# NicholasMilef/UUO-Mocap

Hardware: AMD Instinct MI355X
Metric: mocap frames/sec fitted (300-frame seq, 50 markers) (higher is better)
Workload: dtype f32

## Files before the change

### uuo_mocap_amd/csrc/closure.hip

```cpp
#include <cstddef>
#include <cstdlib>
#include <cstring>
#include <vector>

#include "frame_math.h"
#include "tri_math.h"

#define UUO_STAGE_UPSTREAM 3

struct FinArgs {
  UuoGridHdr h;
  int stage, F;
  uuo_gptr<const float> frame_part;
  uuo_gptr<const float> betas;
  uuo_gptr<const float> o_betas;
  double closs;
  double cpose;
  double cbetas;
  uuo_gptr<float> g_betas;
  uuo_gptr<float> g_z;
  uuo_gptr<float> loss;
  uuo_gptr<const float> dir_betas;
  uuo_gptr<const float> dir_z;
  uuo_gptr<double> stats;
// ... 274 lines not shown
        FIN_REP(12, __double_as_longlong(own1));
        FIN_REP(13, __double_as_longlong(own2));
#pragma unroll
        for (int l = 0; l < 10; ++l) FIN_REP(14 + l, __double_as_longlong((double)gb_local[l]));
#undef FIN_REP
        if constexpr (COHERENT) {
          asm volatile("s_waitcnt vmcnt(0)" ::: "memory");
          __hip_atomic_store(&a.rep_host[10], a.rep_seq, __ATOMIC_RELAXED, __HIP_MEMORY_SCOPE_SYSTEM);
        } else {
          __threadfence_system();
          __hip_atomic_store(&a.rep_host[10], a.rep_seq, __ATOMIC_RELEASE, __HIP_MEMORY_SCOPE_SYSTEM);
        }
      }
    }
  }
}

#ifdef UUO_DEBUG_HOOKS
#define BWD_NSTAMP 12
__device__ unsigned long long g_bwd_stamps[4096 * BWD_NSTAMP];
#define BWD_STAMP(i)                                                                                          \
  do {                                                                                                        \
    if (a.stop == 9 && threadIdx.x == 0 && blockIdx.x < 4096)                                                 \
      g_bwd_stamps[blockIdx.x * BWD_NSTAMP + (i)] = __builtin_amdgcn_s_memtime();                              \
  } while (0)
#else
#define BWD_STAMP(i) do {} while (0)
#endif
__device__ __forceinline__ float gmof_q(float sig2, float s) { return sig2 / (sig2 + s); }

#define BWD_NW 4
#define BWD_SLOTS (BWD_NW * 4)
#ifndef UUO_FIN_FUSED
#define UUO_FIN_FUSED 0
#endif
#if UUO_FIN_FUSED || defined(UUO_DEBUG_HOOKS)
#define UUO_FIN_FUSED_BUILT 1
#define BWD_FP_STORE(i_, v_) \
  __hip_atomic_store(a.frame_part.get() + (size_t)f * UUO_FP + (i_), (float)(v_), __ATOMIC_RELAXED, __HIP_MEMORY_SCOPE_AGENT)
#else
#define UUO_FIN_FUSED_BUILT 0
#define BWD_FP_STORE(i_, v_) a.frame_part[(size_t)f * UUO_FP + (i_)] = (float)(v_)
#endif
enum : unsigned {
  BWD_PART = 1u << 0,
  BWD_ONE_WAVE = 1u << 1,
  BWD_DENSE = 1u << 2,
  BWD_ITEMS = 1u << 3,
  BWD_ROBUST = 1u << 4,
  BWD_ACCEL = 1u << 5,
  BWD_OFFS = 1u << 6,
  BWD_FASSIGN = 1u << 7,
  BWD_FLOOR = 1u << 8,
};
template <unsigned FL>
__device__ __forceinline__ void bwd_body(const BwdArgs& a) {
  constexpr bool PART = (FL & BWD_PART) != 0, DENSE = (FL & BWD_DENSE) != 0, ITEMS = (FL & BWD_ITEMS) != 0;
  constexpr bool ROBUST = (FL & BWD_ROBUST) != 0, ACCEL = (FL & BWD_ACCEL) != 0, OFFS = (FL & BWD_OFFS) != 0;
  constexpr bool FASSIGN = (FL & BWD_FASSIGN) != 0, FLOOR = (FL & BWD_FLOOR) != 0;
  constexpr int NWV = (FL & BWD_ONE_WAVE) ? 1 : BWD_NW;
  static_assert(!FLOOR || (ACCEL && !(FASSIGN && !ITEMS)), "the floor-contact term rides on the temporal instantiations (slot 3 of "
                "the partials, the frames' FrameLds), outside the per-frame vertex table of the one-hot marker closure");
  static_assert(!FASSIGN || (!OFFS && !PART && !DENSE && NWV == BWD_NW), "per-frame vertex ids belong to item mode (the surface "
                "chamfer closure) and to the marker stage's one-hot closure, without latent offsets");
  static_assert(!OFFS || (!PART && !DENSE && NWV == BWD_NW), "the latent marker offsets are built for the marker stage's "
                "sparse kernels only");
  static_assert(!ROBUST || (!DENSE && !ITEMS), "the robust data term is formed on the sparse items (k_bary_fwd for item mode)");
  static_assert(!ACCEL || (!PART && !DENSE && NWV == BWD_NW), "the joint-acceleration term is built for the fitted stages' "
                "sparse kernels (chamfer, marker) only");
  static_assert(!(PART && DENSE), "the part stage's dense sums come through the runtime `pre` pointer");
  static_assert(!ITEMS || (!PART && !DENSE), "item mode belongs to the general sparse kernel");
  static_assert(NWV == BWD_NW || (PART && NWV == 1), "one-wave blocks exist for the part stage only");
  constexpr int NT = NWV * 64, SLOTS = NWV * 4;
  if constexpr (NWV == BWD_NW) __builtin_amdgcn_s_setprio(2);
  __shared__ FrameLds L;
  __shared__ float sA[UUO_NUM_JOINTS * 12];
  __shared__ float spf[UUO_KB];
  __shared__ float w_dA[SLOTS][UUO_NUM_JOINTS * 12];
  __shared__ float w_dpf[PART ? 1 : SLOTS][PART ? 256 : UUO_KB];
  __shared__ float w_red[SLOTS][16];
  __shared__ float sdA[UUO_NUM_JOINTS * 12];
  __shared__ float sdpf[UUO_KB];
  __shared__ float red[16];
  __shared__ float sdGR[UUO_NUM_JOINTS][9], sdGt[UUO_NUM_JOINTS][3], sdJ[UUO_NUM_JOINTS][3], sdR[UUO_NUM_JOINTS][9];
  __shared__ float spsq[UUO_NUM_JOINTS];
  __shared__ float sstat[28][4];
  __shared__ int s_lvl_n[UUO_MAX_DEPTH], s_lvl_j[UUO_MAX_DEPTH][UUO_LEVEL_W], s_lvl_p[UUO_MAX_DEPTH][UUO_LEVEL_W];
  __shared__ int s_nch[UUO_NUM_JOINTS], s_ch[UUO_NUM_JOINTS][4];
  constexpr int ACC_W = 75, ACC_UJ = 5 * ACC_W, ACC_AA = ACC_UJ + 72;
  __shared__ float s_acc[ACCEL ? ACC_AA + 72 : 1];

  const int f = blockIdx.x;
  const int tid = threadIdx.x, wave = tid >> 6, lane = tid & 63;
  const int F = a.F, M = a.M;
  BWD_STAMP(0);
  {
    const UuoTree* tr_ = a.tree;
    if (tid < UUO_MAX_DEPTH) s_lvl_n[tid] = tr_->level_n[tid];
    if (tid < UUO_MAX_DEPTH * UUO_LEVEL_W) {
      (&s_lvl_j[0][0])[tid] = (&tr_->level_j[0][0])[tid];
      (&s_lvl_p[0][0])[tid] = (&tr_->level_p[0][0])[tid];
    }
    if constexpr (NWV >= 4) {
      if (tid >= 64 && tid < 64 + UUO_NUM_JOINTS) s_nch[tid - 64] = tr_->nchild[tid - 64];
      if (tid >= 128 && tid < 128 + UUO_NUM_JOINTS * 4) (&s_ch[0][0])[tid - 128] = (&tr_->child[0][0])[tid - 128];
    } else {
      if (tid < UUO_NUM_JOINTS) s_nch[tid] = tr_->nchild[tid];
      for (int i = tid; i < UUO_NUM_JOINTS * 4; i += NT) (&s_ch[0][0])[i] = (&tr_->child[0][0])[i];
    }
  }
  if (a.frames) {
    constexpr int NW = sizeof(FrameLds) / 4;
    float* dst_l = reinterpret_cast<float*>(&L);
    for (int i = tid; i < NW; i += NT) dst_l[i] = a.frames[(size_t)f * NW + i];
    __syncthreads();
  } else {
    frame_forward(a.src, a.tree, f, L);
  }
  if constexpr (ACCEL) {
    constexpr int NW = sizeof(FrameLds) / 4, GT = offsetof(FrameLds, Gt) / 4;
    for (int i = tid; i < 5 * ACC_W; i += NT) {
      const int t = i / ACC_W, k = i - t * ACC_W, ft = f - 2 + t;
      float v = 0.f;
      if (ft >= 0 && ft < F) v = (k < 72) ? a.frames[(size_t)ft * NW + GT + k] : a.src.trans[(size_t)ft * 3 + (k - 72)];
      s_acc[i] = v;
    }
    if (a.lock_w != 0.f && tid >= NT - 6) {
      const int q = tid - (NT - 6), sft = q / 3, k = (10 + sft) * 3 + (q - sft * 3);
      const float c0 = a.contacts[(size_t)f * 2 + sft];
      s_acc[ACC_UJ + k] = (f >= 1) ? c0 * a.contacts[(size_t)(f - 1) * 2 + sft] : 0.f;
      s_acc[ACC_AA + k] = (f + 1 < F) ? a.contacts[(size_t)(f + 1) * 2 + sft] * c0 : 0.f;
    }
  }
  if (tid < UUO_NUM_JOINTS) frame_skin_matrix(L, tid, sA + tid * 12);
  if (!PART && tid < UUO_KB) {
    float v = 0.f;
    if (tid < UUO_NUM_POSE_FEATS) {
      const int j = 1 + tid / 9, e = tid % 9;
      v = L.R[j][e] - ((e == 0 || e == 4 || e == 8) ? 1.f : 0.f);
    }
    spf[tid] = v;
  }
  for (int i = tid; i < SLOTS * UUO_NUM_JOINTS * 12; i += NT) (&w_dA[0][0])[i] = 0.f;
  for (int i = tid; i < 28 * 4; i += NT) (&sstat[0][0])[i] = 0.f;
  __syncthreads();

  if (a.stop == 1) return;
  BWD_STAMP(1);
  bool use_pre = DENSE;
  if constexpr (PART) use_pre = a.pre.get() != nullptr;
  if (use_pre) {
    if constexpr (PART) {
      const float* pr = a.pre.get() + (size_t)f * UUO_PRE;
      for (int i = tid; i < UUO_NUM_JOINTS * 12; i += NT) {
        const int jj = i / 12, e = i - jj * 12;
        sdA[i] = ((e & 3) == 3) ? pr[16 + jj * 3 + (e >> 2)] : 0.f;
      }
      if (tid < 14) red[tid] = pr[tid];
    } else if constexpr (DENSE) {
      const float* pr = a.pre.get() + (size_t)f * UUO_PREG;
      for (int i = tid; i < UUO_NUM_JOINTS * 12; i += NT) sdA[i] = pr[16 + i];
      if (tid < 4) red[tid] = pr[tid];
      if (tid < UUO_NUM_POSE_FEATS + UUO_NUM_BETAS) {
        float acc = 0.f;
        const float* pp = a.dpf_part.get() + (size_t)f * UUO_KP + tid;
        for (int cb = 0; cb < UUO_DPF_NCB; ++cb) acc += pp[(size_t)cb * F * UUO_KP];
        if (tid < UUO_NUM_POSE_FEATS) sdpf[tid] = acc;
        else red[4 + tid - UUO_NUM_POSE_FEATS] = acc;
      } else if (tid == UUO_NUM_POSE_FEATS + UUO_NUM_BETAS) {
        sdpf[UUO_NUM_POSE_FEATS] = 0.f;
      }
    }
  } else if constexpr (!DENSE) {
  float tr[3] = {0.f, 0.f, 0.f};
  if (a.src.trans) {
    tr[0] = a.src.trans[(size_t)f * 3];
    tr[1] = a.src.trans[(size_t)f * 3 + 1];
    tr[2] = a.src.trans[(size_t)f * 3 + 2];
  }
  {
    const int gq = lane >> 4, sl = lane & 15;
    const int slot = wave * 4 + gq;
    float fk[13];
#pragma unroll
    for (int t = 0; t < 13; ++t) fk[t] = PART ? 0.f : spf[sl + 16 * t];
    const float beta_s = (sl < 10) ? L.beta[sl] : 0.f;
    float acc_pf[13];
#pragma unroll
    for (int t = 0; t < 13; ++t) acc_pf[t] = 0.f;
    float acc_db16 = 0.f, acc_dt16 = 0.f, acc_loss16 = 0.f;
    float* my_dA = &w_dA[slot][0];
    struct Item16 {
      float p[3][13];
      float x0, x1, x2, wgt, d2, vt0, vt1, vt2, st0, st1, st2;
      int4 wi;
      float4 ww;
      float o[OFFS ? 3 : 1];
      bool fl;
    };
    auto fetch16 = [&](int m, Item16& q) {
      const bool in = m < M;
      const int mm = in ? m : 0;
      float wgt = in ? 1.f : 0.f;
      float d2 = 0.f;
      int vi;
      float up0 = 0.f, up1 = 0.f, up2 = 0.f;
      bool fl = false;
      if constexpr (FLOOR) fl = !in && m < M + a.floor_k;
      if (FLOOR && fl) {
        const int kf = m - M;
        vi = a.floor_vids[kf];
        const float* pu = a.floor_up + ((size_t)f * a.floor_k + kf) * 3;
        up0 = pu[0]; up1 = pu[1]; up2 = pu[2];
        wgt = 1.f;
      } else if constexpr (ITEMS) {
        if constexpr (FASSIGN)
          vi = a.assign[(size_t)f * M + mm];
        else
          vi = a.assign[mm];
        const float* pu = a.up_items + ((size_t)f * M + mm) * 3;
        up0 = pu[0]; up1 = pu[1]; up2 = pu[2];
      } else if (a.stage == UUO_STAGE_UPSTREAM) {
        if (mm < a.V) {
          vi = mm;
          if (a.up_verts) {
            const float* pu = a.up_verts + ((size_t)f * a.V + mm) * 3;
            up0 = pu[0]; up1 = pu[1]; up2 = pu[2];
          }
        } else {
          vi = a.tree->extra_vids[mm - a.V];
          const float* pu = a.up_joints + ((size_t)f * 45 + UUO_NUM_JOINTS + (mm - a.V)) * 3;
          up0 = pu[0]; up1 = pu[1]; up2 = pu[2];
        }
      } else if (a.stage == UUO_STAGE_MARKER) {
        wgt *= a.mask[(size_t)f * M + mm];
        if constexpr (FASSIGN) {
          vi = a.assign[(size_t)f * M + mm];
          if (vi < 0) {
// ... 18 lines not shown
      if constexpr (FLOOR) q.fl = fl;
      if (ITEMS || a.stage == UUO_STAGE_UPSTREAM || (FLOOR && fl)) {
        q.x0 = up0; q.x1 = up1; q.x2 = up2;
      } else {
        const float* px = a.markers + ((size_t)f * M + mm) * 3;
        q.x0 = px[0]; q.x1 = px[1]; q.x2 = px[2];
      }
      if constexpr (PART) {
        const float* pc = a.C + ((size_t)f * a.V + vi) * 3;
        q.vt0 = pc[0];
        q.vt1 = pc[1];
        q.vt2 = pc[2];
      } else {
        const float* pt = a.PT + (size_t)vi * 3 * UUO_KB + sl;
#pragma unroll
        for (int c = 0; c < 3; ++c)
#pragma unroll
          for (int t = 0; t < 13; ++t) q.p[c][t] = pt[c * UUO_KB + 16 * t];
        q.vt0 = a.vt[(size_t)vi * 3];
        q.vt1 = a.vt[(size_t)vi * 3 + 1];
        q.vt2 = a.vt[(size_t)vi * 3 + 2];
      }
      const float* ps = a.ST + (size_t)vi * 30 + (sl < 10 ? sl : 0);
      q.st0 = (sl < 10) ? ps[0] : 0.f;
      q.st1 = (sl < 10) ? ps[10] : 0.f;
      q.st2 = (sl < 10) ? ps[20] : 0.f;
      q.wi = *reinterpret_cast<const int4*>(a.Wi + (size_t)vi * 4);
      q.ww = *reinterpret_cast<const float4*>(a.Ww + (size_t)vi * 4);
      if constexpr (OFFS) {
        const float* po = a.offs + (size_t)(mm / a.offs_k) * 3;
        q.o[0] = po[0]; q.o[1] = po[1]; q.o[2] = po[2];
        if (FLOOR && fl) q.o[0] = q.o[1] = q.o[2] = 0.f;
      }
    };
    auto row_sum = [](float v) {
      v += dpp_rot<0x128>(v);
      v += dpp_rot<0x124>(v);
      v += dpp_rot<0x122>(v);
      v += dpp_rot<0x121>(v);
      return v;
    };
    const int rounds = ((FLOOR ? M + a.floor_k : M) + SLOTS - 1) / SLOTS;
    Item16 cur;
    for (int r = 0; r < rounds; ++r) {
      fetch16(slot + SLOTS * r, cur);
      const float wgt = cur.wgt, d2 = cur.d2;
      float vp[3];
      if constexpr (PART) {
        vp[0] = cur.vt0 + row_sum(cur.st0 * beta_s);
        vp[1] = cur.vt1 + row_sum(cur.st1 * beta_s);
        vp[2] = cur.vt2 + row_sum(cur.st2 * beta_s);
      } else {
        float s0 = 0.f, s1 = 0.f, s2 = 0.f;
#pragma unroll
        for (int t = 0; t < 13; ++t) {
          s0 = fmaf(cur.p[0][t], fk[t], s0);
          s1 = fmaf(cur.p[1][t], fk[t], s1);
          s2 = fmaf(cur.p[2][t], fk[t], s2);
        }
        vp[0] = row_sum(s0) + (cur.vt0 + row_sum(cur.st0 * beta_s));
        vp[1] = row_sum(s1) + (cur.vt1 + row_sum(cur.st1 * beta_s));
        vp[2] = row_sum(s2) + (cur.vt2 + row_sum(cur.st2 * beta_s));
      }
      if constexpr (OFFS) {
        vp[0] += cur.o[0];
        vp[1] += cur.o[1];
        vp[2] += cur.o[2];
      }
      float T[12];
#pragma unroll
      for (int e = 0; e < 12; ++e) T[e] = 0.f;
      const int wj[4] = {cur.wi.x, cur.wi.y, cur.wi.z, cur.wi.w};
      const float ww[4] = {cur.ww.x, cur.ww.y, cur.ww.z, cur.ww.w};
#pragma unroll
      for (int n = 0; n < 4; ++n) {
        const float4* pa4 = reinterpret_cast<const float4*>(sA + wj[n] * 12);
        const float4 r0 = pa4[0], r1 = pa4[1], r2 = pa4[2];
        const float w = ww[n];
        T[0] = fmaf(w, r0.x, T[0]); T[1] = fmaf(w, r0.y, T[1]); T[2] = fmaf(w, r0.z, T[2]); T[3] = fmaf(w, r0.w, T[3]);
        T[4] = fmaf(w, r1.x, T[4]); T[5] = fmaf(w, r1.y, T[5]); T[6] = fmaf(w, r1.z, T[6]); T[7] = fmaf(w, r1.w, T[7]);
        T[8] = fmaf(w, r2.x, T[8]); T[9] = fmaf(w, r2.y, T[9]); T[10] = fmaf(w, r2.z, T[10]); T[11] = fmaf(w, r2.w, T[11]);
      }
      const float vx = fmaf(T[2], vp[2], fmaf(T[1], vp[1], T[0] * vp[0])) + T[3] + tr[0];
      const float vy = fmaf(T[6], vp[2], fmaf(T[5], vp[1], T[4] * vp[0])) + T[7] + tr[1];
      const float vz = fmaf(T[10], vp[2], fmaf(T[9], vp[1], T[8] * vp[0])) + T[11] + tr[2];
      const float dx = cur.x0 - vx, dy = cur.x1 - vy, dz = cur.x2 - vz;
      float g[3];
      float loss_item;
      if (ITEMS || a.stage == UUO_STAGE_UPSTREAM || (FLOOR && cur.fl)) {
        loss_item = 0.f;
        g[0] = wgt * cur.x0; g[1] = wgt * cur.x1; g[2] = wgt * cur.x2;
      } else if (a.stage == UUO_STAGE_MARKER) {
        const float rr = sqrtf((dx * dx + dy * dy) + dz * dz);
        const float e = rr - a.d0;
        float lw = wgt, gw = wgt;
        if constexpr (ROBUST) {
          const float q = gmof_q(a.rs2, e * e);
          lw = wgt * q;
          gw = wgt * (q * q);
        }
        loss_item = lw * (e * e);
        const float sc = (rr > 0.f) ? (-a.cg * gw * e / rr) : 0.f;
        g[0] = sc * dx; g[1] = sc * dy; g[2] = sc * dz;
      } else {
        float lw = wgt, gw = wgt;
        if constexpr (ROBUST) {
          const float q = gmof_q(a.rs2, d2);
          lw = wgt * q;
          gw = wgt * (q * q);
        }
        loss_item = lw * d2;
        const float sc = -a.cg * gw;
        g[0] = sc * dx; g[1] = sc * dy; g[2] = sc * dz;
      }
      float dvp[3];
#pragma unroll
      for (int c = 0; c < 3; ++c) dvp[c] = fmaf(T[8 + c], g[2], fmaf(T[4 + c], g[1], T[c] * g[0]));
      if constexpr (OFFS) {
        const int mi = slot + SLOTS * r;
        if (mi < M && sl < 3) a.offs_part[((size_t)f * M + mi) * 3 + sl] = (sl == 0) ? dvp[0] : ((sl == 1) ? dvp[1] : dvp[2]);
      }
      if constexpr (!PART) {
#pragma unroll
        for (int t = 0; t < 13; ++t)
          acc_pf[t] += fmaf(cur.p[2][t], dvp[2], fmaf(cur.p[1][t], dvp[1], cur.p[0][t] * dvp[0]));
      }
      acc_db16 += fmaf(cur.st2, dvp[2], fmaf(cur.st1, dvp[1], cur.st0 * dvp[0]));
      if (sl < 12) {
        const int rr_ = sl >> 2, cc_ = sl & 3;
        const float gr = (rr_ == 0) ? g[0] : ((rr_ == 1) ? g[1] : g[2]);
        const float pc = (cc_ == 0) ? vp[0] : ((cc_ == 1) ? vp[1] : ((cc_ == 2) ? vp[2] : 1.f));
        const float val = gr * pc;
#pragma unroll
        for (int n = 0; n < 4; ++n) my_dA[wj[n] * 12 + sl] += ww[n] * val;
      }
      acc_dt16 += (sl == 0) ? g[0] : ((sl == 1) ? g[1] : g[2]);
      acc_loss16 += loss_item;
    }
    if constexpr (!PART) {
#pragma unroll
      for (int t = 0; t < 13; ++t) w_dpf[slot][sl + 16 * t] = acc_pf[t];
    }
    if (sl == 0) w_red[slot][0] = acc_loss16;
    if (sl < 3) w_red[slot][1 + sl] = acc_dt16;
    if (sl < 10) w_red[slot][4 + sl] = acc_db16;
  }

  if (a.stop == 2) return;
  BWD_STAMP(2);
  __syncthreads();
  BWD_STAMP(3);
  if constexpr (!PART) {
    if (tid < UUO_KB) {
      float acc = w_dpf[0][tid];
#pragma unroll
      for (int w = 1; w < SLOTS; ++w) acc += w_dpf[w][tid];
      sdpf[tid] = acc;
    }
  }
  for (int i = tid; i < UUO_NUM_JOINTS * 12; i += NT) {
    float acc = w_dA[0][i];
#pragma unroll
    for (int w = 1; w < SLOTS; ++w) acc += w_dA[w][i];
    sdA[i] = acc;
  }
  if (tid < 14) {
    float acc = w_red[0][tid];
#pragma unroll
    for (int w = 1; w < SLOTS; ++w) acc += w_red[w][tid];
    red[tid] = acc;
  }
  }
  __syncthreads();

  if (a.stop == 3) return;
  BWD_STAMP(4);
  const UuoTree* tree = a.tree;
  const int j = tid;
  float dpre[9] = {0.f, 0.f, 0.f, 0.f, 0.f, 0.f, 0.f, 0.f, 0.f};
  if (a.dir) {
    if (tid >= 1 && tid < UUO_NUM_JOINTS && a.off_pose >= 0) {
      const float* pd = a.dir + a.off_pose + ((size_t)f * 23 + (tid - 1)) * a.gs_pose;
#pragma unroll
      for (int e = 0; e < 9; ++e) dpre[e] = (e < 6 || a.gs_pose == 9) ? pd[e] : 0.f;
    } else if (tid == 0) {
      if (a.stage == UUO_STAGE_CHAMFER) dpre[0] = a.dir[a.off_z + f];
      if (a.stage == UUO_STAGE_MARKER) {
        const float* pd = a.dir + a.off_root + (size_t)f * a.gs_root;
#pragma unroll
        for (int e = 0; e < 6; ++e) dpre[e] = pd[e];
      }
    } else if (tid >= 32 && tid < 35) {
      dpre[0] = a.dir[a.off_trans + (size_t)f * 3 + (tid - 32)];
    }
  }

  float raw_pre[9] = {0.f, 0.f, 0.f, 0.f, 0.f, 0.f, 0.f, 0.f, 0.f}, po_pre[9] = {0.f, 0.f, 0.f, 0.f, 0.f, 0.f, 0.f, 0.f, 0.f};
  if (!PART && j >= 1 && j < UUO_NUM_JOINTS && a.g_pose) {
    const float* pr = a.raw_pose + ((size_t)f * 23 + (j - 1)) * 9;
#pragma unroll
    for (int e = 0; e < 9; ++e) raw_pre[e] = pr[e];
    if (a.cpose != 0.f) {
      const float* po = a.o_pose + ((size_t)f * 23 + (j - 1)) * 9;
#pragma unroll
      for (int e = 0; e < 9; ++e) po_pre[e] = po[e];
    }
  }
  for (int t = tid; t < UUO_NUM_JOINTS * 12; t += NT) {
    const int jj = t / 12, e = t - jj * 12;
    if (e < 9) {
      const int r = e / 3, c = e - r * 3;
      sdGR[jj][e] = sdA[jj * 12 + r * 4 + c] - sdA[jj * 12 + r * 4 + 3] * L.J[jj][c];
    } else {
      const int r = e - 9;
      float uj = (a.stage == UUO_STAGE_UPSTREAM && a.up_joints) ? a.up_joints[((size_t)f * 45 + jj) * 3 + r] : 0.f;
      if constexpr (ACCEL) {
        const int k = jj * 3 + r;
        float w[5], tw[5];
#pragma unroll
        for (int i = 0; i < 5; ++i) {
          w[i] = s_acc[i * ACC_W + k];
          tw[i] = s_acc[i * ACC_W + 72 + r];
        }
        float ac[3];
#pragma unroll
        for (int i = 0; i < 3; ++i) {
// ... 29 lines not shown
        const int nch = s_nch[jj];
        const int c0 = s_ch[jj][0], c1 = s_ch[jj][1], c2 = s_ch[jj][2], c3 = s_ch[jj][3];
        if (e < 9) {
          const int r = e / 3, aa = e - r * 3;
          float acc = sdGR[jj][e];
#pragma unroll
          for (int ci = 0; ci < 4; ++ci) {
            if (ci < nch) {
              const int c = (ci == 0) ? c0 : ((ci == 1) ? c1 : ((ci == 2) ? c2 : c3));
              float add = fmaf(sdGR[c][r * 3 + 2], L.R[c][aa * 3 + 2],
                               fmaf(sdGR[c][r * 3 + 1], L.R[c][aa * 3 + 1], sdGR[c][r * 3] * L.R[c][aa * 3]));
              add = fmaf(sdGt[c][r], L.J[c][aa] - L.J[jj][aa], add);
              acc += add;
            }
          }
          sdGR[jj][e] = acc;
        } else {
          const int r = e - 9;
          float acc_t = sdGt[jj][r], acc_j = sdJ[jj][r];
#pragma unroll
          for (int ci = 0; ci < 4; ++ci) {
            if (ci < nch) {
              const int c = (ci == 0) ? c0 : ((ci == 1) ? c1 : ((ci == 2) ? c2 : c3));
              acc_t += sdGt[c][r];
              acc_j -= fmaf(L.GR[jj][6 + r], sdGt[c][2], fmaf(L.GR[jj][3 + r], sdGt[c][1], L.GR[jj][r] * sdGt[c][0]));
            }
          }
          sdGt[jj][r] = acc_t;
          sdJ[jj][r] = acc_j;
        }
      } else if (role == 1 && rl < 12 * UUO_LEVEL_W && k < s_lvl_n[d + 1]) {
        const int jj = s_lvl_j[d + 1][k], p = s_lvl_p[d + 1][k];
        if (e < 9) {
          const int aa = e / 3, bb = e - aa * 3;
          sdR[jj][e] = fmaf(L.GR[p][6 + aa], sdGR[jj][6 + bb], fmaf(L.GR[p][3 + aa], sdGR[jj][3 + bb], L.GR[p][aa] * sdGR[jj][bb]));
        } else {
          const int aa = e - 9;
          sdJ[jj][aa] += fmaf(L.GR[p][6 + aa], sdGt[jj][2], fmaf(L.GR[p][3 + aa], sdGt[jj][1], L.GR[p][aa] * sdGt[jj][0]));
        }
      }
     }
      __syncthreads();
    }
  }
  if (tid < 12) {
    if (tid < 9) sdR[0][tid] = sdGR[0][tid];
    else sdJ[0][tid - 9] += sdGt[0][tid - 9];
  }
  __syncthreads();

  BWD_STAMP(6);
  for (int t = tid; t < 240; t += NT) {
    const int jj = t / 10, l = t - jj * 10;
    w_dpf[0][t] = fmaf(tree->JS[jj][2][l], sdJ[jj][2], fmaf(tree->JS[jj][1][l], sdJ[jj][1], tree->JS[jj][0][l] * sdJ[jj][0]));
  }
  __syncthreads();
  if (tid < 10) {
    float acc = red[4 + tid];
    for (int jj = 0; jj < UUO_NUM_JOINTS; ++jj) acc += w_dpf[0][jj * 10 + tid];
    BWD_FP_STORE(4 + tid, acc);
    if (a.stage == UUO_STAGE_UPSTREAM) a.g_betas_frame[(size_t)f * 10 + tid] = acc;
  }
  BWD_STAMP(7);
  if (j >= 1 && j < UUO_NUM_JOINTS) {
    float psq = 0.f;
    if (!PART && a.g_pose) {
      float dR[9], raw[9], gout[9];
#pragma unroll
      for (int e = 0; e < 9; ++e) {
        dR[e] = sdR[j][e] + sdpf[(j - 1) * 9 + e];
        raw[e] = raw_pre[e];
      }
      if (a.src.norm_body) {
        float da[6];
        gs6d_backward(raw, dR, da);
#pragma unroll
        for (int e = 0; e < 6; ++e) gout[e] = da[e];
        gout[6] = gout[7] = gout[8] = 0.f;
      } else {
#pragma unroll
        for (int e = 0; e < 9; ++e) gout[e] = dR[e];
      }
      if (a.cpose != 0.f) {
#pragma unroll
        for (int e = 0; e < 9; ++e) {
          const float diff = raw[e] - po_pre[e];
          gout[e] = fmaf(a.cpose, diff, gout[e]);
          psq = fmaf(diff, diff, psq);
        }
      }
      if constexpr (ACCEL) {
        if (a.lim_g) {
          const unsigned row = ((unsigned)f * 23u + (unsigned)(j - 1)) * 9u;
#pragma unroll
          for (int e = 0; e < 9; ++e) gout[e] += a.lim_g[row + e];
        }
      }
      float* pg = a.g_pose + ((size_t)f * 23 + (j - 1)) * a.gs_pose;
      float sd = 0.f, s1 = 0.f, s2 = 0.f, sm = 0.f;
#pragma unroll
      for (int e = 0; e < 9; ++e) {
        if (e < 6 || a.gs_pose == 9) pg[e] = gout[e];
        sd = fmaf(gout[e], dpre[e], sd);
        s1 += fabsf(gout[e]);
        s2 = fmaf(gout[e], gout[e], s2);
        sm = fmaxf(sm, fabsf(gout[e]));
      }
      sstat[j - 1][0] = sd; sstat[j - 1][1] = s1; sstat[j - 1][2] = s2; sstat[j - 1][3] = sm;
    }
    spsq[j] = psq;
  }
  if (j == 0) {
// ... 64 lines not shown
  if (tid < 4) {
    float acc = 0.f;
    if (tid < 3) {
      for (int w = 0; w < 27; ++w) acc += sstat[w][tid];
    } else {
      for (int w = 0; w < 27; ++w) acc = fmaxf(acc, sstat[w][3]);
    }
    BWD_FP_STORE(16 + tid, acc);
  }
  if (tid == 0) {
    float ps = 0.f;
    for (int jj = 1; jj < UUO_NUM_JOINTS; ++jj) ps += spsq[jj];
    if constexpr (ITEMS) BWD_FP_STORE(0, red[0] + a.item_loss[f]);
    else BWD_FP_STORE(0, red[0]);
    BWD_FP_STORE(2, ps);
    if (a.stage != UUO_STAGE_PART) BWD_FP_STORE(1, 0.f);
  }
  if constexpr (ACCEL) {
    if (tid == 64) {
      float s = 0.f;
      for (int k = 0; k < 72; ++k) s += s_acc[ACC_AA + k];
      float share = a.acc_w * s;
      if (a.lock_w != 0.f) {
        float sl = 0.f;
        for (int k = 30; k < 36; ++k) sl += s_acc[k];
        share += a.lock_w * sl;
      }
      if constexpr (FLOOR) share += a.floor_loss[f];
      if (a.cap_up) share += a.cap_up[(unsigned)a.F * 72u + (unsigned)f];
      if (a.lim_g) share += a.lim_g[(unsigned)a.F * 207u + (unsigned)f];
      BWD_FP_STORE(3, share);
    }
  }
  BWD_STAMP(10);
#if UUO_FIN_FUSED_BUILT
  if constexpr (!PART) {
    if (a.fin_counter) {
      __shared__ unsigned s_arrived;
      asm volatile("s_waitcnt vmcnt(0)" ::: "memory");
      __syncthreads();
      if (tid == 0)
        s_arrived = __hip_atomic_fetch_add(a.fin_counter.get(), 1u, __ATOMIC_RELAXED, __HIP_MEMORY_SCOPE_AGENT);
      __syncthreads();
      if (s_arrived == (unsigned)a.h.gx - 1u) {
        if (tid == 0) __hip_atomic_store(a.fin_counter.get(), 0u, __ATOMIC_RELAXED, __HIP_MEMORY_SCOPE_AGENT);
        finalize_body<NT, true, ACCEL>(a.fin);
      }
    }
  }
#endif
}

#define BWD_WPE3 __attribute__((amdgpu_waves_per_eu(3, 3)))
#define BWD_NO_ATTR
#define BWD_NO_OP (-1)
#define BWD_KERNELS(X, XB)                                                                                                       \
  XB(k_bwd_sparse, 0u, BWD_NW * 64, BWD_WPE3, UUO_OP_BWD, k_bwd_sparse_b)                                                         \
                                      \
  XB(k_bwd_sparse_r, BWD_ROBUST, BWD_NW * 64, BWD_WPE3, UUO_OP_BWD_R, k_bwd_sparse_b_r)                                           \
         \
  X(k_bwd_sparse_t, BWD_ACCEL, BWD_NW * 64, BWD_WPE3, BWD_NO_OP)                                                                  \
  X(k_bwd_sparse_r_t, BWD_ROBUST | BWD_ACCEL, BWD_NW * 64, BWD_WPE3, BWD_NO_OP)                                                   \
       \
  X(k_bwd_sparse_f, BWD_FASSIGN, BWD_NW * 64, BWD_WPE3, BWD_NO_OP)                                                                \
  X(k_bwd_sparse_r_f, BWD_ROBUST | BWD_FASSIGN, BWD_NW * 64, BWD_WPE3, BWD_NO_OP)                                                 \
  X(k_bwd_sparse_t_f, BWD_ACCEL | BWD_FASSIGN, BWD_NW * 64, BWD_WPE3, BWD_NO_OP)                                                  \
  X(k_bwd_sparse_r_t_f, BWD_ROBUST | BWD_ACCEL | BWD_FASSIGN, BWD_NW * 64, BWD_WPE3, BWD_NO_OP)                                   \
                                                  \
  X(k_bwd_dense, BWD_DENSE, BWD_NW * 64, BWD_NO_ATTR, BWD_NO_OP)                                                                  \
                          \
  X(k_bwd_items, BWD_ITEMS, BWD_NW * 64, BWD_NO_ATTR, BWD_NO_OP)                                                                  \
  X(k_bwd_items_t, BWD_ITEMS | BWD_ACCEL, BWD_NW * 64, BWD_NO_ATTR, BWD_NO_OP)                                                    \
                                 \
  X(k_bwd_items_f, BWD_ITEMS | BWD_FASSIGN, BWD_NW * 64, BWD_NO_ATTR, BWD_NO_OP)                                                  \
  X(k_bwd_items_t_f, BWD_ITEMS | BWD_ACCEL | BWD_FASSIGN, BWD_NW * 64, BWD_NO_ATTR, BWD_NO_OP)                                    \
        \
  X(k_bwd_sparse_o, BWD_OFFS, BWD_NW * 64, BWD_WPE3, BWD_NO_OP)                                                                   \
  X(k_bwd_sparse_r_o, BWD_ROBUST | BWD_OFFS, BWD_NW * 64, BWD_WPE3, BWD_NO_OP)                                                    \
  X(k_bwd_sparse_t_o, BWD_ACCEL | BWD_OFFS, BWD_NW * 64, BWD_WPE3, BWD_NO_OP)                                                     \
  X(k_bwd_sparse_r_t_o, BWD_ROBUST | BWD_ACCEL | BWD_OFFS, BWD_NW * 64, BWD_WPE3, BWD_NO_OP)                                      \
  X(k_bwd_items_o, BWD_ITEMS | BWD_OFFS, BWD_NW * 64, BWD_NO_ATTR, BWD_NO_OP)                                                     \
  X(k_bwd_items_t_o, BWD_ITEMS | BWD_ACCEL | BWD_OFFS, BWD_NW * 64, BWD_NO_ATTR, BWD_NO_OP)                                       \
                                                                                   \
  X(k_bwd_sparse_t_fl, BWD_ACCEL | BWD_FLOOR, BWD_NW * 64, BWD_WPE3, BWD_NO_OP)                                                   \
  X(k_bwd_sparse_r_t_fl, BWD_ROBUST | BWD_ACCEL | BWD_FLOOR, BWD_NW * 64, BWD_WPE3, BWD_NO_OP)                                    \
  X(k_bwd_sparse_t_o_fl, BWD_ACCEL | BWD_OFFS | BWD_FLOOR, BWD_NW * 64, BWD_WPE3, BWD_NO_OP)                                      \
  X(k_bwd_sparse_r_t_o_fl, BWD_ROBUST | BWD_ACCEL | BWD_OFFS | BWD_FLOOR, BWD_NW * 64, BWD_WPE3, BWD_NO_OP)                       \
  X(k_bwd_items_t_fl, BWD_ITEMS | BWD_ACCEL | BWD_FLOOR, BWD_NW * 64, BWD_NO_ATTR, BWD_NO_OP)                                     \
  X(k_bwd_items_t_o_fl, BWD_ITEMS | BWD_ACCEL | BWD_OFFS | BWD_FLOOR, BWD_NW * 64, BWD_NO_ATTR, BWD_NO_OP)                        \
  X(k_bwd_items_t_f_fl, BWD_ITEMS | BWD_ACCEL | BWD_FASSIGN | BWD_FLOOR, BWD_NW * 64, BWD_NO_ATTR, BWD_NO_OP)                     \
                                             \
  XB(k_bwd_part1, BWD_PART | BWD_ONE_WAVE, 64, BWD_NO_ATTR, UUO_OP_BWD_PART, k_bwd_part1_b)                                       \
  XB(k_bwd_part, BWD_PART, BWD_NW * 64, BWD_NO_ATTR, UUO_OP_BWD_PART, k_bwd_part_b)                                               \
                                                      \
  XB(k_bwd_part1_r, BWD_PART | BWD_ONE_WAVE | BWD_ROBUST, 64, BWD_NO_ATTR, UUO_OP_BWD_PART_R, k_bwd_part1_b_r)                    \
  XB(k_bwd_part_r, BWD_PART | BWD_ROBUST, BWD_NW * 64, BWD_NO_ATTR, UUO_OP_BWD_PART_R, k_bwd_part_b_r)

#define BWD_ENTRY(name, fl, nt, attr, op) \
  __global__ __launch_bounds__(nt) attr void name(BwdArgs a) { bwd_body<(fl)>(a); }
#define BWD_ENTRY_B(name, fl, nt, attr, op, twin)                                          \
  BWD_ENTRY(name, fl, nt, attr, op)                                                        \
  __global__ __launch_bounds__(nt) attr void twin(const BwdArgs* __restrict__ batch) {     \
    UUO_BATCH_PICK(BwdArgs, batch)                                                         \
    bwd_body<(fl)>(a);                                                                     \
  }
BWD_KERNELS(BWD_ENTRY, BWD_ENTRY_B)

struct BwdKernel {
  unsigned flags;
  int threads;
  int op;
  const char* name;
  void (*kernel)(BwdArgs);
  void (*batch)(const BwdArgs*);
};
#define BWD_ROW(name, fl, nt, attr, op) {(fl), (nt), (op), #name, name, nullptr},
#define BWD_ROW_B(name, fl, nt, attr, op, twin) {(fl), (nt), (op), #name, name, twin},
static const BwdKernel bwd_kernels[] = {BWD_KERNELS(BWD_ROW, BWD_ROW_B)};

struct BwdFacts {
  int stage;
  bool part_cached;
  bool one_wave;
  bool three_corner;
  bool surface;
  bool dense;
  bool robust, temporal, offs, fassign, floor;
};
enum BwdRoute { BWD_ROUTE_PART, BWD_ROUTE_THREE_CORNER, BWD_ROUTE_SURFACE, BWD_ROUTE_DENSE, BWD_ROUTE_GENERAL };
static BwdRoute bwd_route(const BwdFacts& k) {
  if (k.part_cached) return BWD_ROUTE_PART;
  if (k.three_corner) return BWD_ROUTE_THREE_CORNER;
  if (k.surface) return BWD_ROUTE_SURFACE;
  return k.dense ? BWD_ROUTE_DENSE : BWD_ROUTE_GENERAL;
}
static unsigned bwd_flags(const BwdFacts& k) {
  const unsigned r = k.robust ? BWD_ROBUST : 0u, t = k.temporal ? BWD_ACCEL : 0u, o = k.offs ? BWD_OFFS : 0u;
  const unsigned fa = k.fassign ? BWD_FASSIGN : 0u, fl = k.floor ? BWD_FLOOR : 0u;
  switch (bwd_route(k)) {
    case BWD_ROUTE_PART: return BWD_PART | (k.one_wave ? BWD_ONE_WAVE : 0u) | r;
    case BWD_ROUTE_THREE_CORNER: return BWD_ITEMS | t | o | fl;
    case BWD_ROUTE_SURFACE: return BWD_ITEMS | BWD_FASSIGN | t | fl;
    case BWD_ROUTE_DENSE: return BWD_DENSE;
    default: return r | t | o | fa | fl;
  }
}
static int bwd_select(const BwdFacts& k, const BwdKernel** out) {
  const bool refused = (k.fassign && (k.stage != UUO_STAGE_MARKER || k.three_corner || k.offs || k.floor)) ||
                       (bwd_route(k) == BWD_ROUTE_SURFACE && (k.stage != UUO_STAGE_CHAMFER || k.dense));
  const unsigned fl = bwd_flags(k);
  *out = nullptr;
  if (!refused)
    for (const BwdKernel& row : bwd_kernels)
      if (row.flags == fl) *out = &row;
  UUO_REQUIRE(*out, "closure: no backward kernel for stage " + std::to_string(k.stage) + (k.part_cached ? " part_cached" : "") +
                        (k.one_wave ? " one_wave" : "") + (k.three_corner ? " three_corner" : "") + (k.surface ? " surface" : "") +
                        (k.dense ? " dense" : "") + (k.robust ? " robust" : "") + (k.temporal ? " temporal" : "") +
                        (k.offs ? " offs" : "") + (k.fassign ? " fassign" : "") + (k.floor ? " floor" : ""));
  return 0;
}

struct BaryFwdArgs {
  uuo_gptr<const float> PT, ST, vt, Ww;
  uuo_gptr<const int> Wi;
  uuo_gptr<const UuoTree> tree;
  int V, F, M;
  UuoPoseSrc src;
  uuo_gptr<const float> markers, mask;
  uuo_gptr<const int> assign3;
  uuo_gptr<const float> bary;
  float cg, d0;
// ... 998 lines not shown
    std::memset(&b, 0, sizeof(b));
    b.PT = m->PT; b.ST = m->ST; b.vt = m->vt; b.Ww = m->Ww; b.Wi = m->Wi; b.tree = m->tree;
    b.V = m->V; b.F = F; b.M = M;
    b.src = src;
    b.markers = p->d_markers;
    b.mask = fit->mask;
    b.corners = fit->surf_corners;
    b.cg = a.cg;
    b.d0 = fit->surface_distance;
    b.rs2 = a.rs2;
    b.frames = fit->frames;
    b.up_items = items;
    b.item_loss = item_loss;
    b.bary = fit->surf_bary;
    hipLaunchKernelGGL(robust ? k_surf_fwd_r : k_surf_fwd, dim3(F), dim3(BWD_NW * 64), 0, s, b);
    launch_side_terms();
    a.M = 3 * M;
    a.assign = fit->surf_corners;
    a.up_items = items;
    a.item_loss = item_loss;
    a.frames = fit->frames;
  } else if (route == BWD_ROUTE_DENSE) {
    rc = uuo_launch_soft_chamfer(s, F, M, m->V, p->d_markers, fit->verts, fit->mask, fit->mask_sum, fit->nn, p->w_data, p->w_soft,
                                 p->soft_tau, fit->soft_sm, fit->soft_gV, fit->dense->pre, UUO_PREG,
                                 ((m->VP / 16) <= 512 && M <= 512) ? fit->bbox : nullptr);
    if (rc) return rc;
    rc = uuo_dense_backward(m, s, F, fit->pfaT, fit->A, fit->soft_gV, fit->dense, have_vp);
    if (rc) return rc;
    a.pre = fit->dense->pre;
    a.dpf_part = fit->dense->part;
  } else {
    UUO_REQUIRE(!soft, "closure: the soft-assignment part closure runs on the cached pose blend only");
#ifndef UUO_FIN_FUSED
#define UUO_FIN_FUSED 1
#endif
    const int fin_unfused = UUO_ENV_INT("UUO_FIN_UNFUSED", !UUO_FIN_FUSED);
    if (!fin_unfused && !offs) {
      a.fin = fa;
      a.fin_counter = reinterpret_cast<unsigned*>(fit->scalars + 32);
      fin_fused = true;
    }
    if (temporal) {
      if (p->stage == UUO_STAGE_MARKER) {
        rc = uuo_launch_pose_prep(m, s, F, src, fit->pfaT, fit->A, nullptr, fit->frames);
        if (rc) return rc;
        a.frames = fit->frames;
      }
      launch_side_terms();
    }
  }
  const BwdKernel* bk = nullptr;
  rc = bwd_select(k, &bk);
  if (rc) return rc;
  if (bk->op == BWD_NO_OP || !uuo_record(bk->op, F, (bk->flags & BWD_PART) ? bk->threads / 64 : 1, a))
    hipLaunchKernelGGL((bk->kernel), dim3(F), dim3(bk->threads), 0, s, a);
  UUO_HIP_CHECK(hipGetLastError());
  if (!fin_fused) {
    if (offs)
      hipLaunchKernelGGL(temporal ? k_finalize_to : k_finalize_o, dim3(1), dim3(1024), 0, s, fa, oa);
    else if (temporal)
      hipLaunchKernelGGL(k_finalize_t, dim3(1), dim3(1024), 0, s, fa);
    else if (!uuo_record(UUO_OP_FIN, 1, 1, fa))
      hipLaunchKernelGGL(k_finalize, dim3(1), dim3(1024), 0, s, fa);
    UUO_HIP_CHECK(hipGetLastError());
  }

  return 0;
}

extern "C" int uuo_closure_eval(uuo_fit_t* fit, void* stream, const uuo_problem_t* p, const float* d_x, float* d_loss,
                                float* d_grad, int32_t* d_nn_idx) {
  int rc = validate_problem(fit, p);
  if (rc) return rc;
  UUO_REQUIRE(d_x && d_loss && d_grad, "uuo_closure_eval: null x/loss/grad");
  hipStream_t s = (hipStream_t)stream;
  rc = uuo_ensure_mask(fit, s, p);
  if (rc) return rc;
  return uuo_closure_eval_impl(fit, s, p, d_x, d_loss, d_grad, d_nn_idx, nullptr, nullptr);
}

extern "C" int uuo_time_closure(uuo_fit_t* fit, void* stream, const uuo_problem_t* p, const float* d_x, int iters,
                                int dominant_only, float* ms_per_eval) {
  int rc = validate_problem(fit, p);
  if (rc) return rc;
  UUO_REQUIRE(d_x && ms_per_eval && iters > 0, "uuo_time_closure: bad arguments");
  hipStream_t s = (hipStream_t)stream;
  const StageLayout lay = problem_layout(p);
  float* loss = fit->scalars + 8;
  float* grad = fit->vecs;
  rc = uuo_ensure_mask(fit, s, p);
  if (rc) return rc;
  const UuoPoseSrc src = stage_pose_src(p, lay, d_x);
  rc = dominant_only ? closure_forward(fit, s, p, src, false) : uuo_closure_eval_impl(fit, s, p, d_x, loss, grad, nullptr, nullptr, nullptr);
  if (rc) return rc;
  if (dominant_only) {
    float total = 0.f;
    const bool k3 = dominant_only == 2;
    for (int i = 0; i < 10; ++i) {
      rc = k3 ? uuo_launch_skin16(fit->model, s, p->F, fit->pfa16, fit->A, src.trans, fit->verts, fit->bbox)
              : uuo_launch_skin(fit->model, s, p->F, fit->pfaT, fit->A, src.trans, fit->verts, fit->bbox);
      if (rc) return rc;
    }
    for (int i = 0; i < iters; ++i) {
      UUO_HIP_CHECK(hipEventRecord(fit->ev0, s));
      rc = k3 ? uuo_launch_skin16(fit->model, s, p->F, fit->pfa16, fit->A, src.trans, fit->verts, fit->bbox)
              : uuo_launch_skin(fit->model, s, p->F, fit->pfaT, fit->A, src.trans, fit->verts, fit->bbox);
// ... 204 lines not shown
```

Measured before the change: 1491.

## Alias backward-kernel LDS phases in a union and cap sparse VGPRs

The backward kernel's shared arrays now live in a union so that arrays used in different phases share the same bytes. Loop-phase buffers (sA, spf, w_dA) overlap with reduce and tail buffers (sdA, sdpf, w_dpf, joint tail, JS scratch), which cuts LDS per block. The pose-feature vector is reloaded from LDS inside the item loop rather than kept in 13 registers, and the w_dpf reduction moves after the main reduction with extra barriers. The sparse kernels also get an 80-VGPR cap, aiming at better occupancy at the cost of more LDS reads, extra syncs and possible spills; the old layout stays available behind a debug env flag.

```diff
diff --git a/uuo_mocap_amd/csrc/closure.hip b/uuo_mocap_amd/csrc/closure.hip
--- a/uuo_mocap_amd/csrc/closure.hip
+++ b/uuo_mocap_amd/csrc/closure.hip
@@ -350,7 +350,44 @@
   BWD_OFFS = 1u << 6,
   BWD_FASSIGN = 1u << 7,
   BWD_FLOOR = 1u << 8,
+  BWD_WIDE = 1u << 9,
 };
+constexpr int BWD_NA = UUO_NUM_JOINTS * 12;
+struct BwdLdsTail {
+  float sdGR[UUO_NUM_JOINTS][9], sdGt[UUO_NUM_JOINTS][3], sdJ[UUO_NUM_JOINTS][3], sdR[UUO_NUM_JOINTS][9];
+  float spsq[UUO_NUM_JOINTS];
+  float sstat[28][4];
+};
+template <int SLOTS>
+struct BwdLdsPhased {
+  union {
+    struct {
+      float sA[BWD_NA], spf[UUO_KB];
+      float w_dA[SLOTS][BWD_NA];
+    };
+    struct {
+      float sA_unused[BWD_NA], sdpf[UUO_KB];
+      float sdA[BWD_NA];
+      union {
+        float w_dpf[SLOTS][UUO_KB];
+        struct {
+          BwdLdsTail t;
+          float js[240];
+        };
+      };
+    };
+  };
+};
+static_assert(offsetof(BwdLdsPhased<BWD_SLOTS>, sdpf) == offsetof(BwdLdsPhased<BWD_SLOTS>, spf) &&
+              offsetof(BwdLdsPhased<BWD_SLOTS>, sdA) == offsetof(BwdLdsPhased<BWD_SLOTS>, w_dA) &&
+              offsetof(BwdLdsPhased<BWD_SLOTS>, w_dpf) == offsetof(BwdLdsPhased<BWD_SLOTS>, w_dA) + sizeof(float) * BWD_NA &&
+              sizeof(BwdLdsPhased<BWD_SLOTS>) == sizeof(float) * (BWD_NA + UUO_KB + BWD_SLOTS * BWD_NA),
+              "REDUCE and TAIL fit into LOOP's bytes: sdA is row 0 of w_dA, w_dpf and the tail's arrays start at row 1");
+template <bool PHASED, class A, class B>
+__device__ __forceinline__ auto& bwd_lds_pick(A& phased, B& own) {
+  if constexpr (PHASED) return phased;
+  else return own;
+}
 template <unsigned FL>
 __device__ __forceinline__ void bwd_body(const BwdArgs& a) {
   constexpr bool PART = (FL & BWD_PART) != 0, DENSE = (FL & BWD_DENSE) != 0, ITEMS = (FL & BWD_ITEMS) != 0;
@@ -371,18 +408,33 @@
   static_assert(NWV == BWD_NW || (PART && NWV == 1), "one-wave blocks exist for the part stage only");
   constexpr int NT = NWV * 64, SLOTS = NWV * 4;
   if constexpr (NWV == BWD_NW) __builtin_amdgcn_s_setprio(2);
+  constexpr bool PHASED = !PART && !(FL & BWD_WIDE), PF_LDS = PHASED && !DENSE && !ITEMS;
   __shared__ FrameLds L;
-  __shared__ float sA[UUO_NUM_JOINTS * 12];
-  __shared__ float spf[UUO_KB];
-  __shared__ float w_dA[SLOTS][UUO_NUM_JOINTS * 12];
-  __shared__ float w_dpf[PART ? 1 : SLOTS][PART ? 256 : UUO_KB];
+  __shared__ BwdLdsPhased<SLOTS> S;
+  __shared__ float sA_[UUO_NUM_JOINTS * 12];
+  __shared__ float spf_[UUO_KB];
+  __shared__ float w_dA_[SLOTS][UUO_NUM_JOINTS * 12];
+  __shared__ float w_dpf_[PART ? 1 : SLOTS][PART ? 256 : UUO_KB];
+  __shared__ float sdA_[UUO_NUM_JOINTS * 12];
+  __shared__ float sdpf_[UUO_KB];
+  __shared__ float sdGR_[UUO_NUM_JOINTS][9], sdGt_[UUO_NUM_JOINTS][3], sdJ_[UUO_NUM_JOINTS][3], sdR_[UUO_NUM_JOINTS][9];
+  __shared__ float spsq_[UUO_NUM_JOINTS];
+  __shared__ float sstat_[28][4];
+  auto& sA = bwd_lds_pick<PHASED>(S.sA, sA_);
+  auto& spf = bwd_lds_pick<PHASED>(S.spf, spf_);
+  auto& w_dA = bwd_lds_pick<PHASED>(S.w_dA, w_dA_);
+  auto& w_dpf = bwd_lds_pick<PHASED>(S.w_dpf, w_dpf_);
+  auto& sdA = bwd_lds_pick<PHASED>(S.sdA, sdA_);
+  auto& sdpf = bwd_lds_pick<PHASED>(S.sdpf, sdpf_);
+  auto& sdGR = bwd_lds_pick<PHASED>(S.t.sdGR, sdGR_);
+  auto& sdGt = bwd_lds_pick<PHASED>(S.t.sdGt, sdGt_);
+  auto& sdJ = bwd_lds_pick<PHASED>(S.t.sdJ, sdJ_);
+  auto& sdR = bwd_lds_pick<PHASED>(S.t.sdR, sdR_);
+  auto& spsq = bwd_lds_pick<PHASED>(S.t.spsq, spsq_);
+  auto& sstat = bwd_lds_pick<PHASED>(S.t.sstat, sstat_);
+  float* const sjs = PHASED ? &S.js[0] : &w_dpf_[0][0];
   __shared__ float w_red[SLOTS][16];
-  __shared__ float sdA[UUO_NUM_JOINTS * 12];
-  __shared__ float sdpf[UUO_KB];
   __shared__ float red[16];
-  __shared__ float sdGR[UUO_NUM_JOINTS][9], sdGt[UUO_NUM_JOINTS][3], sdJ[UUO_NUM_JOINTS][3], sdR[UUO_NUM_JOINTS][9];
-  __shared__ float spsq[UUO_NUM_JOINTS];
-  __shared__ float sstat[28][4];
   __shared__ int s_lvl_n[UUO_MAX_DEPTH], s_lvl_j[UUO_MAX_DEPTH][UUO_LEVEL_W], s_lvl_p[UUO_MAX_DEPTH][UUO_LEVEL_W];
   __shared__ int s_nch[UUO_NUM_JOINTS], s_ch[UUO_NUM_JOINTS][4];
   constexpr int ACC_W = 75, ACC_UJ = 5 * ACC_W, ACC_AA = ACC_UJ + 72;
@@ -440,7 +492,9 @@
     spf[tid] = v;
   }
   for (int i = tid; i < SLOTS * UUO_NUM_JOINTS * 12; i += NT) (&w_dA[0][0])[i] = 0.f;
-  for (int i = tid; i < 28 * 4; i += NT) (&sstat[0][0])[i] = 0.f;
+  if constexpr (!PHASED) {
+    for (int i = tid; i < 28 * 4; i += NT) (&sstat[0][0])[i] = 0.f;
+  }
   __syncthreads();
 
   if (a.stop == 1) return;
@@ -481,7 +535,7 @@
     const int slot = wave * 4 + gq;
     float fk[13];
 #pragma unroll
-    for (int t = 0; t < 13; ++t) fk[t] = PART ? 0.f : spf[sl + 16 * t];
+    for (int t = 0; t < 13; ++t) fk[t] = (PART || PF_LDS) ? 0.f : spf[sl + 16 * t];
     const float beta_s = (sl < 10) ? L.beta[sl] : 0.f;
     float acc_pf[13];
 #pragma unroll
@@ -606,6 +660,12 @@
         vp[2] = cur.vt2 + row_sum(cur.st2 * beta_s);
       } else {
         float s0 = 0.f, s1 = 0.f, s2 = 0.f;
+        if constexpr (PF_LDS) {
+          int sl_r = sl;
+          asm volatile("" : "+v"(sl_r));
+#pragma unroll
+          for (int t = 0; t < 13; ++t) fk[t] = spf[sl_r + 16 * t];
+        }
 #pragma unroll
         for (int t = 0; t < 13; ++t) {
           s0 = fmaf(cur.p[0][t], fk[t], s0);
@@ -691,20 +751,19 @@
       acc_dt16 += (sl == 0) ? g[0] : ((sl == 1) ? g[1] : g[2]);
       acc_loss16 += loss_item;
     }
-    if constexpr (!PART) {
+    if constexpr (!PART && !PHASED) {
 #pragma unroll
       for (int t = 0; t < 13; ++t) w_dpf[slot][sl + 16 * t] = acc_pf[t];
     }
     if (sl == 0) w_red[slot][0] = acc_loss16;
     if (sl < 3) w_red[slot][1 + sl] = acc_dt16;
     if (sl < 10) w_red[slot][4 + sl] = acc_db16;
-  }
 
   if (a.stop == 2) return;
   BWD_STAMP(2);
   __syncthreads();
   BWD_STAMP(3);
-  if constexpr (!PART) {
+  if constexpr (!PART && !PHASED) {
     if (tid < UUO_KB) {
       float acc = w_dpf[0][tid];
 #pragma unroll
@@ -724,8 +783,24 @@
     for (int w = 1; w < SLOTS; ++w) acc += w_red[w][tid];
     red[tid] = acc;
   }
+  if constexpr (PHASED) {
+    __syncthreads();
+#pragma unroll
+    for (int t = 0; t < 13; ++t) w_dpf[slot][sl + 16 * t] = acc_pf[t];
+    __syncthreads();
+    if (tid < UUO_KB) {
+      float acc = w_dpf[0][tid];
+#pragma unroll
+      for (int w = 1; w < SLOTS; ++w) acc += w_dpf[w][tid];
+      sdpf[tid] = acc;
+    }
+  }
+  }
   }
   __syncthreads();
+  if constexpr (PHASED) {
+    for (int i = tid; i < 28 * 4; i += NT) (&sstat[0][0])[i] = 0.f;
+  }
 
   if (a.stop == 3) return;
   BWD_STAMP(4);
@@ -861,12 +936,12 @@
   BWD_STAMP(6);
   for (int t = tid; t < 240; t += NT) {
     const int jj = t / 10, l = t - jj * 10;
-    w_dpf[0][t] = fmaf(tree->JS[jj][2][l], sdJ[jj][2], fmaf(tree->JS[jj][1][l], sdJ[jj][1], tree->JS[jj][0][l] * sdJ[jj][0]));
+    sjs[t] = fmaf(tree->JS[jj][2][l], sdJ[jj][2], fmaf(tree->JS[jj][1][l], sdJ[jj][1], tree->JS[jj][0][l] * sdJ[jj][0]));
   }
   __syncthreads();
   if (tid < 10) {
     float acc = red[4 + tid];
-    for (int jj = 0; jj < UUO_NUM_JOINTS; ++jj) acc += w_dpf[0][jj * 10 + tid];
+    for (int jj = 0; jj < UUO_NUM_JOINTS; ++jj) acc += sjs[jj * 10 + tid];
     BWD_FP_STORE(4 + tid, acc);
     if (a.stage == UUO_STAGE_UPSTREAM) a.g_betas_frame[(size_t)f * 10 + tid] = acc;
   }
@@ -1037,12 +1112,13 @@
 }
 
 #define BWD_WPE3 __attribute__((amdgpu_waves_per_eu(3, 3)))
+#define BWD_WPE3_V160 __attribute__((amdgpu_waves_per_eu(3, 3), amdgpu_num_vgpr(80)))
 #define BWD_NO_ATTR
 #define BWD_NO_OP (-1)
 #define BWD_KERNELS(X, XB)                                                                                                       \
-  XB(k_bwd_sparse, 0u, BWD_NW * 64, BWD_WPE3, UUO_OP_BWD, k_bwd_sparse_b)                                                         \
+  XB(k_bwd_sparse, 0u, BWD_NW * 64, BWD_WPE3_V160, UUO_OP_BWD, k_bwd_sparse_b)                                                   \
                                       \
-  XB(k_bwd_sparse_r, BWD_ROBUST, BWD_NW * 64, BWD_WPE3, UUO_OP_BWD_R, k_bwd_sparse_b_r)                                           \
+  XB(k_bwd_sparse_r, BWD_ROBUST, BWD_NW * 64, BWD_WPE3_V160, UUO_OP_BWD_R, k_bwd_sparse_b_r)                                     \
          \
   X(k_bwd_sparse_t, BWD_ACCEL, BWD_NW * 64, BWD_WPE3, BWD_NO_OP)                                                                  \
   X(k_bwd_sparse_r_t, BWD_ROBUST | BWD_ACCEL, BWD_NW * 64, BWD_WPE3, BWD_NO_OP)                                                   \
@@ -1102,6 +1178,15 @@
 #define BWD_ROW(name, fl, nt, attr, op) {(fl), (nt), (op), #name, name, nullptr},
 #define BWD_ROW_B(name, fl, nt, attr, op, twin) {(fl), (nt), (op), #name, name, twin},
 static const BwdKernel bwd_kernels[] = {BWD_KERNELS(BWD_ROW, BWD_ROW_B)};
+#ifdef UUO_DEBUG_HOOKS
+#define BWD_WIDE_KERNELS(X)                                                          \
+  X(k_bwd_sparse_wide, BWD_WIDE, BWD_NW * 64, BWD_WPE3, BWD_NO_OP)                    \
+  X(k_bwd_sparse_r_wide, BWD_WIDE | BWD_ROBUST, BWD_NW * 64, BWD_WPE3, BWD_NO_OP)     \
+  X(k_bwd_sparse_t_wide, BWD_WIDE | BWD_ACCEL, BWD_NW * 64, BWD_WPE3, BWD_NO_OP)      \
+  X(k_bwd_sparse_r_t_wide, BWD_WIDE | BWD_ROBUST | BWD_ACCEL, BWD_NW * 64, BWD_WPE3, BWD_NO_OP)
+BWD_WIDE_KERNELS(BWD_ENTRY)
+static const BwdKernel bwd_wide_kernels[] = {BWD_WIDE_KERNELS(BWD_ROW)};
+#endif
 
 struct BwdFacts {
   int stage;
@@ -2206,6 +2291,16 @@
   const BwdKernel* bk = nullptr;
   rc = bwd_select(k, &bk);
   if (rc) return rc;
+#ifdef UUO_DEBUG_HOOKS
+  if (UUO_ENV_INT("UUO_BWD_WIDE_LDS", 0)) {
+    const BwdKernel* wide = nullptr;
+    for (const BwdKernel& row : bwd_wide_kernels)
+      if (row.flags == (bk->flags | BWD_WIDE)) wide = &row;
+    UUO_REQUIRE(wide && !uuo_recorder, std::string("closure: UUO_BWD_WIDE_LDS has no form of ") + bk->name +
+                                           (uuo_recorder ? " inside a lock-step batch" : ""));
+    bk = wide;
+  }
+#endif
   if (bk->op == BWD_NO_OP || !uuo_record(bk->op, F, (bk->flags & BWD_PART) ? bk->threads / 64 : 1, a))
     hipLaunchKernelGGL((bk->kernel), dim3(F), dim3(bk->threads), 0, s, a);
   UUO_HIP_CHECK(hipGetLastError());
```

After: 1540, median of 6. +3.3%, better.
